# wheaton5/cellector

Measured on AMD Instinct MI355X. Metric: cell x locus log-likelihood evals/sec over full EM iterations (EM iters/sec in em_iters_per_s), higher is better.
Workload: dtype f64

## Files before the change

### cellector_amd/csrc/kernels_tiled.hip

```cpp
#include <hip/hip_ext.h>

#include "tiled.h"

__device__ __constant__ uint8_t T_A_OF[T_NCODE] = {1, 0, 2, 1, 0, 3, 2, 1, 0, 4, 3, 2, 1, 0};
__device__ __constant__ uint8_t T_R_OF[T_NCODE] = {0, 1, 0, 1, 2, 0, 1, 2, 3, 0, 1, 2, 3, 4};

struct ab_src_t {
    const double *s_alt, *s_ref, *alt_min, *ref_min;
    const uint8_t *mask;
    double2 *ab_out;
    double *xl_counters;
    uint32_t *d_counters, *tile_work;
    uint32_t n_work;
};
template <bool PAIRS>
__global__ __launch_bounds__(64 * TB_PARTS) void k_build_tables(uint64_t L, uint32_t nj, const double2 *__restrict__ ab,
                                                                const double *__restrict__ lf, double *__restrict__ tab,
                                                                ab_src_t src)
{
    if (src.s_alt && blockIdx.x == 0) {
        if (threadIdx.x < LC_COUNTERS) src.xl_counters[threadIdx.x] = 0.0;
        if (threadIdx.x < 8) src.d_counters[threadIdx.x] = 0u;
        for (uint32_t i = threadIdx.x; i < src.n_work; i += blockDim.x) src.tile_work[i] = 0u;
    }
    const int part = threadIdx.x >> 6;
    const uint64_t t = (uint64_t)blockIdx.x * 64 + (threadIdx.x & 63);
    if (t >= (uint64_t)nj * T_BL) return;
    const uint64_t chunk = t / T_BL, slot = t % T_BL;
    const uint64_t l = chunk * T_BLU + slot;
    double2 p = make_double2(-1.0, -1.0);
    if (slot < T_BLU && l < L) {
        if (src.s_alt) {
            p.x = (src.s_alt[l] + 1.0) - src.alt_min[l];
            p.y = (src.s_ref[l] + 1.0) - src.ref_min[l];
            if (!src.mask[l]) p.x = p.y = -1.0;
            if (part == 0) src.ab_out[l] = p;
        } else {
            p = ab[l];
        }
    }
    const bool live = p.x >= 0.0;
    double *row = tab + chunk * TAB_ELEMS + slot * T_LROW;
#define TB_PMF(W, A, R) row[W] = live ? dm_log_bb_pmf(lf, p.x, p.y, A, R) : 0.0
#define TB_EXP(N) row[T_NCODE + N - 1] = (PAIRS && live) ? dm_expected_log_pmf(lf, p.x, p.y, N) : 0.0
    switch (part) {
    case 0: TB_EXP(4u); TB_PMF(0, 1u, 0u); break;
    case 1: TB_EXP(3u); TB_PMF(1, 0u, 1u); break;
    case 2: TB_EXP(2u); TB_PMF(2, 2u, 0u); TB_PMF(3, 1u, 1u); break;
    case 3: TB_EXP(1u); TB_PMF(4, 0u, 2u); TB_PMF(5, 3u, 0u); break;
    case 4: TB_PMF(6, 2u, 1u); TB_PMF(7, 1u, 2u); TB_PMF(8, 0u, 3u); TB_PMF(9, 4u, 0u); break;
    default: TB_PMF(10, 3u, 1u); TB_PMF(11, 2u, 2u); TB_PMF(12, 1u, 3u); TB_PMF(13, 0u, 4u); break;
    }
#undef TB_PMF
#undef TB_EXP
}

#ifndef TILE_ABL
#define TILE_ABL 0
#endif
#ifndef TILE_PFD
#define TILE_PFD 2
#endif
#ifndef TILE_PFD_T2
#define TILE_PFD_T2 2
#endif
#ifndef TILE_PINNED
#define TILE_PINNED 1
#endif
#if TILE_ABL == 7
#define TILE_BARRIER() do { } while (0)
#else
#define TILE_BARRIER() asm volatile("s_waitcnt lgkmcnt(0)\n\ts_barrier" ::: "memory")
#endif

struct __attribute__((packed, aligned(4))) tile_u4 { uint32_t x, y, z, w; };

template <bool EXPECTED, int T_SB, class G = geo_reg>
__global__ __launch_bounds__(T_THREADS, 4) void k_tile_ll(uint32_t nb, uint32_t nj, uint32_t cpg, uint32_t groups,
                                                          uint32_t n_cols, uint32_t *__restrict__ work ,
                                                          const uint16_t *__restrict__ thdr,
                                                          const uint16_t *__restrict__ tiles,
                                                          const double *__restrict__ tab, uint64_t npad,
                                                          double *__restrict__ part_ll, double *__restrict__ part_ell)
{
    using tab_t = typename std::conditional<EXPECTED, double2, double>::type;
    constexpr uint32_t TAB_U = G::LROW * G::BL * sizeof(double) / 16;
    constexpr int NP = (TAB_U + T_THREADS - 1) / T_THREADS;
    static_assert(NP == 6, "table prefetch registers are written out by hand");
    __shared__ __attribute__((aligned(16))) double s_tab[G::LROW * G::BL];
    static_assert(G::LROW * G::BL % 2 == 0, "whole 16-byte units");
    __shared__ tab_t s_acc[T_SB * T_BC];
    __shared__ uint32_t s_col;
    const uint32_t tid = threadIdx.x, wv = tid >> 6, lane = tid & 63;
    const uint32_t g = blockIdx.x % groups;
    const uint32_t j0 = g * cpg, j1 = min(nj, j0 + cpg);
    if (j0 >= j1) return;
  for (;;) {
    if (tid == 0) s_col = atomicAdd(&work[g], 1u);
    __syncthreads();
    const uint32_t col = s_col;
    if (col >= n_cols) break;
    const uint32_t b0 = col * T_SB;
#pragma unroll
    for (int s = 0; s < T_SB; s++) {
        if constexpr (EXPECTED) s_acc[s * T_BC + tid] = make_double2(0.0, 0.0);
        else s_acc[s * T_BC + tid] = 0.0;
    }

    double2 p_t0, p_t1, p_t2, p_t3, p_t4, p_t5;
#define TABLE_PREFETCH(J)                                                                                        \
    do {                                                                                                         \
        const double2 *src__ = reinterpret_cast<const double2 *>(tab) + (uint64_t)(J) * TAB_U + tid;             \
        p_t0 = src__[0];                                                                                         \
        p_t1 = src__[T_THREADS];                                                                                 \
        p_t2 = src__[2 * T_THREADS];                                                                             \
        p_t3 = src__[3 * T_THREADS];                                                                             \
        p_t4 = src__[4 * T_THREADS];                                                                             \
        p_t5 = src__[5 * T_THREADS];                      \
    } while (0)

    struct row_t { tile_u4 lo, hi; uint32_t k; uint64_t base; };
    const uint32_t wv_s = (uint32_t)__builtin_amdgcn_readfirstlane((int)wv);
#define HDR_LOAD(H, J, S)            \
    do {                                                                                                         \
         \
         \
         \
        const uint32_t rot__ = (wv_s + 8u * ((uint32_t)(S) >> 1)) & 15u, sl__ = ((S) & 1u) ? 15u - rot__ : rot__; \
        if (TILE_ABL != 9 || first_rows)  \
        (H) = reinterpret_cast<const uint4 *>(thdr + ((uint64_t)min(b0 + (uint32_t)(S), nb - 1) * nj + (TILE_ABL == 10 ? j0 : (J))) * T_HDR)[sl__]; \
    } while (0)
#define ROW_LOAD(E, H)                                                                                           \
    do {                                                                                                         \
        (E).k = (SKIP_EMPTY && (H).w) ? 0u : (H).z;  \
        (E).base = ((uint64_t)(H).y << 32) | (H).x;                                                              \
         \
         \
        const char *sb__ = reinterpret_cast<const char *>(tiles + (E).base);                                     \
        const uint32_t off__ = __umul24(lane, ((H).z + 1u) * 2u);                      \
        if ((!(TILE_ABL == 2 || TILE_ABL == 9) || first_rows) && !(SKIP_EMPTY && (H).w)) {  \
            (E).lo = *reinterpret_cast<const tile_u4 *>(sb__ + off__);                                           \
            (E).hi = *reinterpret_cast<const tile_u4 *>(sb__ + ((H).z > 7u ? 16u : 0u) + off__);                 \
        }                                                                                                        \
    } while (0)

    constexpr bool SKIP_EMPTY = G::NLO != 1;
    constexpr uint32_t PFD = T_SB == 4 ? (uint32_t)(G::NLO == 1 ? TILE_PFD : TILE_PFD_T2) : 2u;
    static_assert(PFD >= 2 && PFD <= 4, "row buffers");
    uint4 h0, h1, h2, h3;
    row_t e0, e1, e2, e3;
    bool first_rows = true;
    TABLE_PREFETCH(j0);
    __builtin_amdgcn_sched_barrier(0);
#define HDR_STEP(H, T) HDR_LOAD(H, min(j0 + (uint32_t)(T) / T_SB, j1 - 1), (uint32_t)(T) % T_SB)
    HDR_STEP(h0, 0);
    HDR_STEP(h1, 1);
    if constexpr (PFD >= 3) HDR_STEP(h2, 2);
    if constexpr (PFD == 4) HDR_STEP(h3, 3);
    ROW_LOAD(e0, h0);
    ROW_LOAD(e1, h1);
    if constexpr (PFD >= 3) ROW_LOAD(e2, h2);
    if constexpr (PFD == 4) ROW_LOAD(e3, h3);
    HDR_STEP(h0, PFD);
    HDR_STEP(h1, PFD + 1);
    if constexpr (PFD >= 3) HDR_STEP(h2, PFD + 2);
    if constexpr (PFD == 4) HDR_STEP(h3, PFD + 3);
#undef HDR_STEP
    first_rows = false;

#if TILE_ABL == 1 || TILE_ABL == 5
#define TILE_LOOKUP(V, E16) do { if constexpr (EXPECTED) V = make_double2((double)(E16), 1.0); else V = (double)(E16); } while (0)
#elif TILE_ABL == 4
#define TILE_LOOKUP(V, E16)                                                                                      \
    do {                                                                                                         \
        const uint32_t b__ = (((E16) >> 4) & 127u) * 32u + (lane & 31u), c__ = (((E16) >> 5) & 127u) * 32u + (lane & 31u); \
        if constexpr (EXPECTED) V = make_double2(s_tab[b__], s_tab[c__ + 4096u]);                                \
        else V = s_tab[b__];                                                                                     \
    } while (0)
#else
#define TILE_LOOKUP(V, E16)                                                                                      \
    do {                                                                                                         \
        const uint32_t b__ = (((E16) >> G::SHIFT) & G::SMASK) * G::LROW;                                         \
        if constexpr (EXPECTED) V = make_double2(s_tab[b__ + ((E16) & G::CMASK)], s_tab[b__ + G::NCODE + ((E16) >> 14)]); \
        else V = s_tab[b__ + ((E16) & G::CMASK)];                                                                \
    } while (0)
#endif
#define TILE_RD(V, KK)                                                                                           \
    tab_t V;                                                                                                     \
    do {                                                                                                         \
        const uint32_t idx__ = (((KK) + 1) & 1) ? (w__[((KK) + 1) >> 1] >> 16) : (w__[((KK) + 1) >> 1] & 0xffffu); \
        TILE_LOOKUP(V, idx__);                                                                                   \
    } while (0)
#define TILE_ADD(V)                                                                                              \
    do {                                                                                                         \
        if constexpr (EXPECTED) { a_ll__ += (V).x; a_el__ += (V).y; }                                            \
        else a_ll__ += (V);                                                                                      \
    } while (0)
#if TILE_PINNED
#define TILE_PIN(V)                                                                                              \
    do {                                                                                                         \
        if constexpr (EXPECTED) asm volatile("" : "+v"((V).x), "+v"((V).y) : : "memory");                        \
        else asm volatile("" : "+v"(V) : : "memory");                                                            \
    } while (0)
#else
#define TILE_PIN(V) do { } while (0)
#endif
#define TILE_LEVEL(KA, KB, PA, PB, BODY)                                                                         \
    if (K__ > (KA)) {                                                                                            \
        TILE_RD(v##KA, KA); TILE_RD(v##KB, KB);                                                                  \
        TILE_PIN(PA); TILE_PIN(PB);                                                                              \
        TILE_ADD(PA); TILE_ADD(PB);                                                                              \
        BODY                                                                                                     \
    } else { TILE_ADD(PA); TILE_ADD(PB); }
#define TILE_STEP(S, E, H)                                                                                       \
    do {                                                                                                         \
         \
        const uint32_t w__[8] = {(E).lo.x, (E).lo.y, (E).lo.z, (E).lo.w, (E).hi.x, (E).hi.y, (E).hi.z, (E).hi.w}; \
        const uint32_t K__ = (uint32_t)__builtin_amdgcn_readfirstlane((int)(E).k);        \
        const uint64_t cur_base__ = (E).base;                                                                    \
        const uint32_t cell__ = w__[0] & 0xffffu;                                                                \
              \
        ROW_LOAD(E, H);                                                                                          \
        HDR_LOAD(H, min(j + ((S) + 2 * PFD) / T_SB, j1 - 1), ((S) + 2 * PFD) % T_SB);                            \
         \
          \
        if (!(SKIP_EMPTY && K__ == 0u)) {                                                                        \
        tab_t acc__;                                                                                             \
        if constexpr (TILE_ABL == 8) { if constexpr (EXPECTED) acc__ = make_double2(0.0, 0.0); else acc__ = 0.0; }        \
        else acc__ = s_acc[(S) * T_BC + (TILE_ABL == 6 ? tid : cell__)];                                         \
        double a_ll__ = 0.0, a_el__ = 0.0;                                                                       \
          \
        TILE_RD(v0, 0);                                                                                          \
        if (K__ > 1) {                                                                                           \
            TILE_RD(v1, 1); TILE_RD(v2, 2);                                                                      \
            TILE_PIN(v0);                                                                                        \
            TILE_ADD(v0);                                                                                        \
            TILE_LEVEL(3, 4, v1, v2,                                                                             \
            TILE_LEVEL(5, 6, v3, v4,                                                                             \
            TILE_LEVEL(7, 8, v5, v6,                                                                             \
            TILE_LEVEL(9, 10, v7, v8,                                                                            \
            TILE_LEVEL(11, 12, v9, v10,                                                                          \
            TILE_LEVEL(13, 14, v11, v12,                                                                         \
                TILE_ADD(v13); TILE_ADD(v14);                                                                    \
                for (uint32_t k = T_NE; k < K__; k++) {  \
                    tab_t v__;                                                                                   \
                    TILE_LOOKUP(v__, (uint32_t)(tiles + cur_base__ + lane * (K__ + 1u))[k + 1]);                 \
                    TILE_ADD(v__);                                                                               \
                } ))))))                                                                                         \
        } else TILE_ADD(v0);                                                                                     \
         \
         \
        if constexpr (EXPECTED) { acc__.x += a_ll__; acc__.y += a_el__; }                                        \
        else acc__ += a_ll__;                                                                                    \
        if (TILE_ABL != 8 || a_ll__ == 12345.678) s_acc[(S) * T_BC + (TILE_ABL == 6 ? tid : cell__)] = acc__;   \
        }                                                                                                        \
    } while (0)

    static_assert(T_SB == 2 || T_SB == 4, "even and odd steps use different pipeline buffers");
#if TILE_ABL == 3 || TILE_ABL == 5 || TILE_ABL == 7
#define TILE_STAGE_IF if (j == j0)
#define TILE_NEXT_TABLE() do { } while (0)
#else
#define TILE_STAGE_IF
#define TILE_NEXT_TABLE() TABLE_PREFETCH(min(j + 1, j1 - 1))
#endif
#define TILE_STAGE()                                                                                             \
    do {                                                                                                         \
// ... 236 lines not shown
                den *= fab;
                fa += isa ? 1.0 : 0.0;
                fb += isa ? 0.0 : 1.0;
                fab += 1.0;
            }
            lp = (lf[n] - lf[a] - lf[r]) + log(num * ov_rcp(den));
        } else {
            lp = ov_slow_log_pmf(lf, p.x, p.y, a, r);
        }
        s += lp;
        if (EXPECTED) e += ev;
    }
    s = group16_sum(s);
    if (EXPECTED) e = group16_sum(e);
    if (in && j == 0) {
        o_ll[row] = s;
        if (EXPECTED) o_ell[row] = e;
    }
}

template <bool EXPECTED>
__global__ __launch_bounds__(256) void k_t2_tables(uint32_t n_pairs, const uint32_t *__restrict__ plist ,
                                                   uint32_t n_sec, const uint32_t *__restrict__ slist ,
                                                   uint32_t gp, const double2 *__restrict__ ab, const double *__restrict__ lf,
                                                   double *__restrict__ tab2)
{
    if (blockIdx.x < gp) {
        const uint32_t i = blockIdx.x * 256 + threadIdx.x;
        if (i >= n_pairs) return;
        const uint32_t key = plist[i], l = key >> 5, c2 = key & 31u;
        const uint32_t n = 5u + (c2 >= 6u) + (c2 >= 13u) + (c2 >= 21u), r = c2 - t2_code(n, 0u), a = n - r;
        const double2 p = ab[l];
        double v = 0.0;
        if (p.x >= 0.0) {
            double num = 1.0, den = 1.0, fa = p.x, fb = p.y, fab = p.x + p.y;
#pragma unroll
            for (uint32_t k = 0; k < T2_NMAX; ++k) {
                const bool on = k < n, isa = k < a;
                num *= on ? (isa ? fa : fb) : 1.0;
                den *= on ? fab : 1.0;
                fa += isa ? 1.0 : 0.0;
                fb += (on && !isa) ? 1.0 : 0.0;
                fab += 1.0;
            }
            v = (lf[n] - lf[a] - lf[r]) + log(num / den);
        }
        tab2[(uint64_t)l * T2_ROW + t2_pos(n, r)] = v;
    } else if (EXPECTED) {
        const uint32_t i = (blockIdx.x - gp) * 256 + threadIdx.x;
        if (i >= n_sec) return;
        const uint32_t key = slist[i], l = key >> 3, sec = key & 7u;
        const uint32_t n = 5u + (sec >= 1u) + (sec >= 2u) + (sec >= 4u);
        const double2 p = ab[l];
        tab2[(uint64_t)l * T2_ROW + sec * 8u] = p.x >= 0.0 ? ov_expected_rec(p.x, p.y, n) : 0.0;
    }
}

template <bool EXPECTED, class G>
__global__ __launch_bounds__(256) void k_t2c_tables(uint64_t L, uint32_t gp, const double2 *__restrict__ ab, const double *__restrict__ lf,
                                                    double *__restrict__ tabc)
{
    constexpr uint64_t ELEMS = (uint64_t)G::LROW * G::BL;
    if (blockIdx.x < gp) {
        const uint64_t i = (uint64_t)blockIdx.x * 256 + threadIdx.x;
        const uint64_t l = i / G::NCODE;
        if (l >= L) return;
        const uint32_t c2 = (uint32_t)(i % G::NCODE);
        const uint32_t n = 5u + (c2 >= 6u) + (c2 >= 13u) + (c2 >= 21u), r = c2 - t2_code(n, 0u), a = n - r;
        const double2 p = ab[l];
        double v = 0.0;
        if (p.x >= 0.0) {
            double num = 1.0, den = 1.0, fa = p.x, fb = p.y, fab = p.x + p.y;
#pragma unroll
            for (uint32_t k = 0; k < T2_NMAX; ++k) {
                const bool on = k < n, isa = k < a;
                num *= on ? (isa ? fa : fb) : 1.0;
                den *= on ? fab : 1.0;
                fa += isa ? 1.0 : 0.0;
                fb += (on && !isa) ? 1.0 : 0.0;
                fab += 1.0;
            }
            v = (lf[n] - lf[a] - lf[r]) + log(num / den);
        }
        tabc[(l / G::BLU) * ELEMS + (l % G::BLU) * G::LROW + c2] = v;
    } else if (EXPECTED) {
        constexpr uint32_t NE = G::NHI - G::NLO + 1;
        const uint64_t i = (uint64_t)(blockIdx.x - gp) * 256 + threadIdx.x;
        const uint64_t l = i / NE;
        if (l >= L) return;
        const uint32_t n = G::NLO + (uint32_t)(i % NE);
        const double2 p = ab[l];
        tabc[(l / G::BLU) * ELEMS + (l % G::BLU) * G::LROW + G::NCODE + (n - G::NLO)] = p.x >= 0.0 ? ov_expected_rec(p.x, p.y, n) : 0.0;
    }
}

template <bool EXPECTED>
__global__ __launch_bounds__(256) void k_t2_tile_add(uint64_t n_rows, uint32_t groups, uint64_t npad, const double *__restrict__ part_ll,
                                                     const double *__restrict__ part_ell, double *__restrict__ o_ll,
                                                     double *__restrict__ o_ell)
{
    const uint64_t row = (uint64_t)blockIdx.x * 256 + threadIdx.x;
    if (row >= n_rows) return;
    double s = 0.0, e = 0.0;
    for (uint32_t g = 0; g < groups; g++) {
        s += part_ll[(uint64_t)g * npad + row];
        if (EXPECTED) e += part_ell[(uint64_t)g * npad + row];
    }
    o_ll[row] += s;
    if (EXPECTED) o_ell[row] += e;
}

template <bool EXPECTED>
__global__ __launch_bounds__(64) void k_t2_cell(uint64_t n_rows, const uint64_t *__restrict__ ell_ptr, const uint64_t *__restrict__ ell,
                                                const double *__restrict__ tab2, double *__restrict__ o_ll, double *__restrict__ o_ell)
{
  const uint64_t n_grp = (n_rows + 63) >> 6;
  for (uint64_t grp = blockIdx.x; grp < n_grp; grp += gridDim.x) {
    const uint64_t row = grp * 64 + threadIdx.x;
    if (row >= n_rows) continue;
    double s = 0.0, e = 0.0;
    const uint64_t base = ell_ptr[grp] + (row & 63), end = ell_ptr[grp + 1];
    constexpr int U = 4;
    for (uint64_t i = base; i < end; i += (uint64_t)U * 64) {
        uint64_t en[U];
        double lp[U], ev[U];
#pragma unroll
        for (int u = 0; u < U; u++) en[u] = i + (uint64_t)u * 64 < end ? ell[i + (uint64_t)u * 64] : OVF_PAD;
#pragma unroll
        for (int u = 0; u < U; u++) {
            const uint32_t r = ENT_REF(en[u]), n = ENT_ALT(en[u]) + r;
            const bool ok = en[u] != OVF_PAD && t2_total(n);
#ifdef T2_ABL
            const uint64_t at = (uint64_t)(ENT_IDX(en[u]) & 1023u) * T2_ROW + t2_pos(ok ? n : T2_NMIN, ok ? r : 0u);
#else
            const uint64_t at = (uint64_t)ENT_IDX(en[u]) * T2_ROW + t2_pos(ok ? n : T2_NMIN, ok ? r : 0u);
#endif
            lp[u] = ok ? tab2[at] : 0.0;
            if (EXPECTED) ev[u] = ok ? tab2[at & ~7ull] : 0.0;
        }
#pragma unroll
        for (int u = 0; u < U; u++) {
            s += lp[u];
            if (EXPECTED) e += ev[u];
        }
    }
    o_ll[row] = s;
    if (EXPECTED) o_ell[row] = e;
  }
}

__global__ __launch_bounds__(256) void k_t2_minority(const uint32_t *__restrict__ tc, int valid, uint64_t nloc,
                                                     const uint32_t *__restrict__ minlist, const uint32_t *__restrict__ chg,
                                                     const uint64_t *__restrict__ ovf_ptr, const uint64_t *__restrict__ ovf_ent,
                                                     uint32_t *__restrict__ cnt2)
{
    const uint32_t n_a = valid ? tc[1] : tc[0], n = valid ? n_a + tc[2] : n_a;
    const uint32_t j = threadIdx.x % LF_LANES;
    const uint32_t ng = gridDim.x * (256 / LF_LANES);
    for (uint32_t k = (blockIdx.x * 256 + threadIdx.x) / LF_LANES; k < n; k += ng) {
        const uint32_t cell = !valid ? minlist[k] : k < n_a ? chg[k] : chg[nloc - 1 - (k - n_a)];
        const uint32_t inc = k < n_a ? 1u : ~0u;
        for (uint64_t i = ovf_ptr[cell] + j, end = ovf_ptr[cell + 1]; i < end; i += LF_LANES) {
            const uint64_t en = ovf_ent[i];
            const uint32_t r = ENT_REF(en), t = ENT_ALT(en) + r;
            if (t2_total(t)) atomicAdd(&cnt2[(uint64_t)ENT_IDX(en) * T2_CSTRIDE + t2_code(t, r)], inc);
        }
    }
}

__global__ __launch_bounds__(256) void k_ovx_values(uint64_t n_ovx, const uint32_t *__restrict__ ovx_locus, const uint64_t *__restrict__ ovx_ent,
                                                    const double2 *__restrict__ ab, const double *__restrict__ lf, double *__restrict__ lp_out)
{
    const uint64_t i = (uint64_t)blockIdx.x * 256 + threadIdx.x;
    if (i >= n_ovx) return;
    const uint64_t en = ovx_ent[i];
// ... 366 lines not shown
        s_len[tid] = p_n;
        __syncthreads();
        LR_PREFETCH(kb + LR_THREADS);
        constexpr int SPW = 64 / LR_GROUP;
        constexpr int NQ = 16;
        for (uint32_t q0 = 0; q0 < 64 / SPW; q0 += NQ) {
            uint32_t e[NQ];
#pragma unroll
            for (int u = 0; u < NQ; u++) {
                const uint32_t seg = wv * 64 + (q0 + u) * SPW + grp;
                e[u] = gl < s_len[seg] ? (uint32_t)c4r[s_beg[seg] + gl] : 0xffffu;
            }
#pragma unroll
            for (int u = 0; u < NQ; u++) LR_COUNT(e[u]);
            for (int u = 0; u < NQ; u++) {
                const uint32_t seg = wv * 64 + (q0 + u) * SPW + grp;
                const uint32_t sn = s_len[seg];
                const uint64_t sb = s_beg[seg];
                for (uint32_t j = gl + LR_GROUP; j < sn; j += LR_GROUP) {
                    const uint32_t x = (uint32_t)c4r[sb + j];
                    LR_COUNT(x);
                }
            }
        }
        __syncthreads();
    }
#undef LR_PREFETCH
#undef LR_COUNT
    __syncthreads();
    const uint64_t nl = min((uint64_t)LR_LOCI, L - l0);
    uint32_t *dst = reinterpret_cast<uint32_t *>(reinterpret_cast<uint16_t *>(hist_min) + ((uint64_t)sub * L + l0) * 16);
    for (uint32_t i = tid; i < nl * 8; i += LR_THREADS) {
        const uint32_t lo = i >> 3, c0 = (i & 7u) * 2u;
        uint32_t v = 0;
#pragma unroll
        for (uint32_t h = 0; h < 2; h++) {
            const uint32_t code = c0 + h, idx = code * LR_ROW + lo;
            if (code < (uint32_t)T_NCODE) v |= ((s_hist[idx >> 1] >> ((idx & 1u) * 16u)) & 0xffffu) << (16u * h);
        }
        dst[i] = v;
    }
}

template <bool INLINE_OVF>
__global__ __launch_bounds__(256) void k_locus_finalize(uint64_t L, int locus_mode, int valid, uint64_t nloc, uint32_t n_sub, uint32_t sub_cap,
                                                        const uint32_t *__restrict__ tc,
                                                        const uint32_t *__restrict__ hist_min, uint32_t *__restrict__ tally,
                                                        const uint32_t *__restrict__ flag_bits,
                                                        const uint32_t *__restrict__ hist_all,
                                                        const double *__restrict__ tab, uint32_t tab_stride,
                                                        const uint8_t *__restrict__ mask,
                                                        const uint64_t *__restrict__ ovc_ptr ,
                                                        const uint64_t *__restrict__ ovc_ent,
                                                        const double *__restrict__ ovf_lp ,
                                                        const double *__restrict__ otab, const double *__restrict__ lf,
                                                        const double2 *__restrict__ ab, double *__restrict__ out,
                                                        const uint32_t *__restrict__ cnt2 ,
                                                        const uint32_t *__restrict__ hist_all2, const uint32_t *__restrict__ pmask2,
                                                        const double *__restrict__ tab2,
                                                        uint8_t *__restrict__ mask_next ,
                                                        uint32_t *__restrict__ n_filtered)
{
    const TallyPlan tp = tally_plan(locus_mode, valid, tc, nloc, n_sub, sub_cap);
    const uint32_t n_planes = tp.s_a + tp.s_r;
    const uint32_t j = threadIdx.x % LF_LANES;
    const uint64_t l_raw = ((uint64_t)blockIdx.x * 256 + threadIdx.x) / LF_LANES;
    const bool in = l_raw < L;
    const uint64_t l = in ? l_raw : L - 1;
    const bool live = mask[l] != 0;
    uint64_t obeg = 0, oend = 0;
    if (ovc_ptr) { obeg = ovc_ptr[l]; oend = ovc_ptr[l + 1]; }
    double cmin = 0.0, cmaj = 0.0;
    uint32_t nmin = 0;
    uint64_t amin = 0, rmin = 0;
    if (j < T_NCODE) {
        uint32_t cnt = tp.fresh ? 0u : tally[l * 16 + j];
        if (n_planes) {
            const uint16_t *h16 = reinterpret_cast<const uint16_t *>(hist_min);
            for (uint32_t p = 0; p < tp.s_a; p++) cnt += h16[((uint64_t)p * L + l) * 16 + j];
            for (uint32_t p = tp.s_a; p < n_planes; p++) cnt -= h16[((uint64_t)p * L + l) * 16 + j];
        }
        if (in && (n_planes || tp.fresh)) tally[l * 16 + j] = cnt;
        const uint32_t h_all = hist_all[l * T_NCODE + j];
        const double t_code = tab[(l / T_BLU) * TAB_ELEMS + (l % T_BLU) * T_LROW + j];
        amin = (uint64_t)cnt * T_A_OF[j];
        rmin = (uint64_t)cnt * T_R_OF[j];
        if (live) {
            nmin = cnt;
            cmin = (double)cnt * t_code;
            cmaj = (double)(h_all - cnt) * t_code;
        }
    }
    if (cnt2) {
        const uint32_t pm = pmask2[l];
#pragma unroll
        for (uint32_t h = 0; h < 2; h++) {
            const uint32_t c2 = j + h * LF_LANES;
            if (!((pm >> c2) & 1u)) continue;
            const uint32_t h_all = hist_all2[l * T2_CSTRIDE + c2];
            const uint32_t cnt = cnt2[l * T2_CSTRIDE + c2];
            const uint32_t n2 = 5u + (c2 >= 6u) + (c2 >= 13u) + (c2 >= 21u), r2 = c2 - t2_code(n2, 0u);
            const double t_code = tab2[l * T2_ROW + t2_pos(n2, r2)];
            amin += (uint64_t)cnt * (n2 - r2);
            rmin += (uint64_t)cnt * r2;
            if (live) {
                nmin += cnt;
                cmin += (double)cnt * t_code;
                cmaj += (double)(h_all - cnt) * t_code;
            }
        }
    }
    const double *orow = otab + l * OV_ROW;
    for (uint64_t i0 = obeg + j; i0 < oend; i0 += 4 * LF_LANES) {
        uint64_t en[4];
        double lp[4];
        uint32_t w[4];
#pragma unroll
        for (int u = 0; u < 4; u++) {
            const uint64_t i = i0 + (uint64_t)u * LF_LANES;
            en[u] = i < oend ? ovc_ent[i] : ~0ull;
            lp[u] = (!INLINE_OVF && i < oend) ? ovf_lp[i] : 0.0;
        }
#pragma unroll
        for (int u = 0; u < 4; u++) w[u] = en[u] != ~0ull ? flag_bits[ENT_IDX(en[u]) >> 5] : 0u;
#pragma unroll
        for (int u = 0; u < 4; u++) {
            if (!INLINE_OVF) break;
            lp[u] = 0.0;
            if (en[u] == ~0ull || !live) continue;
            const uint32_t a = ENT_ALT(en[u]), r = ENT_REF(en[u]), n = a + r;
            if (n == 0) lp[u] = 0.0;
            else if (n < (uint32_t)OV_NT)
                lp[u] = (lf[n] - lf[a] - lf[r]) + (orow[a] + orow[OV_NT + r] - orow[2 * OV_NT + n]);
            else {
                const double2 p = ab[l];
                lp[u] = ov_slow_log_pmf(lf, p.x, p.y, a, r);
            }
        }
#pragma unroll
        for (int u = 0; u < 4; u++) {
            if (en[u] == ~0ull) continue;
            const bool minority = ((w[u] >> (ENT_IDX(en[u]) & 31)) & 1u) != 0;
            if (minority) { amin += ENT_ALT(en[u]); rmin += ENT_REF(en[u]); }
            if (live) {
                if (minority) { cmin += lp[u]; nmin++; } else cmaj += lp[u];
            }
        }
    }
    cmin = group16_sum(cmin);
    cmaj = group16_sum(cmaj);
    nmin = group16_sum(nmin);
    amin = group16_sum(amin);
    rmin = group16_sum(rmin);
    if (in && j == 0) {
        out[LB_CONTRIB_MIN * L + l] = cmin;
        out[LB_CONTRIB_MAJ * L + l] = cmaj;
        out[LB_CELLS_MIN * L + l] = (double)nmin;
        out[LB_ALT_MIN * L + l] = (double)amin;
        out[LB_REF_MIN * L + l] = (double)rmin;
        if (mask_next) {
            const double fn = (double)nmin;
            const double per_cell = fn != 0.0 ? cmin / fn : 0.0;
            uint8_t m = mask[l];
            if (per_cell < -80.0) {
                m = 0;
                atomicAdd(n_filtered, 1u);
            }
// ... 493 lines not shown
```

### cellector_amd/csrc/kernels_tiled_build.hip

```cpp
#include "tiled.h"

__device__ __forceinline__ uint64_t row_lower_bound(const uint64_t *__restrict__ ent, uint64_t lo, uint64_t hi, uint32_t locus)
{
    while (lo < hi) {
        const uint64_t mid = (lo + hi) >> 1;
        if (ENT_IDX(ent[mid]) < locus) lo = mid + 1; else hi = mid;
    }
    return lo;
}

template <class G>
__device__ __forceinline__ bool geo_take(uint64_t e)
{
    const uint32_t n = ENT_ALT(e) + ENT_REF(e);
    return n - G::NLO <= G::NHI - G::NLO;
}
template <class G>
__device__ __forceinline__ uint16_t geo_encode(uint64_t e, uint32_t j)
{
    const uint32_t r = ENT_REF(e), n = ENT_ALT(e) + r;
    const uint32_t code = G::NLO == 1 ? ent_code(e) : t2_code(n, r);
    return (uint16_t)(((n - G::NLO) << 14) | ((ENT_IDX(e) - j * G::BLU) << G::SHIFT) | code);
}
template <bool FILL, class G = geo_reg>
// ... 16 lines not shown
    if (cl < T_BC / 64) s_kmax[cl] = 0;
    uint64_t lo = 0, hi = 0;
    uint32_t len = 0;
    if (row < nloc) {
        const uint64_t beg = csr_ptr[row], end = csr_ptr[row + 1];
        if (toff) {
            lo = beg + toff[row * (nj + 1) + j];
            hi = beg + toff[row * (nj + 1) + j + 1];
        } else {
            lo = row_lower_bound(csr_ent, beg, end, j * G::BLU);
            hi = row_lower_bound(csr_ent, lo, end, (j + 1u) * G::BLU);
        }
        for (uint64_t i = lo; i < hi; i++) len += geo_take<G>(csr_ent[i]) ? 1u : 0u;
    }
    __syncthreads();
    const uint32_t bin = min(len, (uint32_t)TB_BINS - 1u);
    uint32_t within = 0;
    {
        unsigned long long todo = ~0ull;
        while (todo) {
            const int src = __ffsll((long long)todo) - 1;
            const uint32_t v = (uint32_t)__shfl((int)bin, src, 64);
            const unsigned long long m = __ballot(bin == v);
            if (bin == v) within = (uint32_t)__popcll(m & ((1ull << lane) - 1ull));
            if ((int)lane == src) s_cnt[wv][v] = (uint32_t)__popcll(m);
            todo &= ~m;
        }
    }
    __syncthreads();
    if (cl < TB_BINS) {
        uint32_t tot = 0;
        for (int w = 0; w < T_BC / 64; w++) tot += s_cnt[w][cl];
        uint32_t inc = tot;
#pragma unroll
        for (int off = 1; off < 64; off <<= 1) {
            const uint32_t o = __shfl_up(inc, off, 64);
            if ((int)cl >= off) inc += o;
        }
        s_base[cl] = inc - tot;
    }
    __syncthreads();
    uint32_t rank = s_base[bin] + within;
    for (uint32_t w = 0; w < wv; w++) rank += s_cnt[w][bin];
    const uint32_t dw = rank >> 6, dl = rank & 63;
    atomicMax(&s_kmax[dw], len);
    __syncthreads();
    if (cl == 0) {
        uint32_t acc = 0;
        for (int w = 0; w < T_BC / 64; w++) {
            s_sbase[w] = acc;
            acc += 64u * ((s_kmax[w] | 1u) + 1u);
        }
        s_sbase[T_BC / 64] = acc;
    }
    __syncthreads();
    if (!FILL) {
        if (cl == 0) tile_elems[t] = (uint64_t)s_sbase[T_BC / 64];
        return;
    }
    const uint64_t tbase = tile_elems[t];
    uint16_t *hp = thdr + t * T_HDR;
    if (cl < T_BC / 64) {
        uint32_t *hd = reinterpret_cast<uint32_t *>(hp) + 4 * cl;
        const uint64_t first = tbase + s_sbase[cl];
        hd[0] = (uint32_t)first;
        hd[1] = (uint32_t)(first >> 32);
        hd[2] = s_kmax[cl] | 1u;
        hd[3] = s_kmax[cl] == 0u;
    }
    const uint32_t K = s_kmax[dw] | 1u;
    uint16_t *dst = tiles + tbase + s_sbase[dw] + dl * (K + 1u);
    dst[0] = (uint16_t)cl;
    uint32_t k = 0;
    for (uint64_t i = lo; i < hi; i++) {
        const uint64_t e = csr_ent[i];
        if (geo_take<G>(e)) dst[1 + k++] = geo_encode<G>(e, j);
    }
    for (; k < K; k++) dst[1 + k] = (uint16_t)(G::BLU << G::SHIFT);
}

#define TBO_ROUNDS 4
__device__ __forceinline__ void tbo_banks(uint32_t e, uint32_t *a, uint32_t *b)
{
    const uint32_t base = ((e >> 4) & 1023u) * (uint32_t)T_LROW;
    *a = (base + (e & 15u)) & 31u;
    *b = (base + (uint32_t)T_NCODE + (e >> 14)) & 31u;
}
__device__ uint32_t tile_lane_assign(uint16_t *slice , uint32_t Kw, uint32_t lane, uint32_t cnt, uint32_t *scr)
{
#define TLA_SYNC() asm volatile("s_waitcnt lgkmcnt(0)" ::: "memory")
    const uint32_t cls = (uint32_t)slice[lane * (Kw + 1u)] & 15u;
    const unsigned long long lt = (1ull << lane) - 1ull;
    uint32_t t = 0;
#pragma unroll
    for (uint32_t c = 0; c < 16u; c++) {
        const unsigned long long m = __ballot(cls == c);
        if (c < cls) t += (uint32_t)__popcll(m);
        else if (c == cls) t += (uint32_t)__popcll(m & lt);
    }
    const uint32_t g = t & 3u, pp = ((t >> 2) + ((g & 1u) ? 8u : 0u)) & 15u;
    const uint32_t l0 = pp < 4u ? pp : (pp < 8u ? pp + 8u : pp + 12u);
    const uint32_t l1 = pp < 8u ? pp + 4u : (pp < 12u ? pp + 8u : pp + 16u);
    const uint32_t dst = ((g & 1u) ? l1 : l0) + ((g & 2u) ? 32u : 0u);
    scr[dst] = lane;
    scr[64 + dst] = cnt;
    TLA_SYNC();
    const uint32_t src = scr[lane], cnt_new = scr[64 + lane];
    for (uint32_t k = 0; k <= Kw; k++) {
        const uint16_t v = slice[src * (Kw + 1u) + k];
        TLA_SYNC();
        slice[lane * (Kw + 1u) + k] = v;
        TLA_SYNC();
    }
    return cnt_new;
#undef TLA_SYNC
}

#define TBO_WIN 4
__device__ void tile_bank_order(uint16_t *row , uint32_t K, uint32_t cnt ,
                                uint32_t lane, uint32_t *scr )
{
    const uint32_t h = lane >> 5;
    uint32_t *ld_a = scr + h * 64, *ld_b = ld_a + 32, *win_a = scr + 128 + h * 64, *win_b = win_a + 32;
#define TBO_SYNC() asm volatile("s_waitcnt lgkmcnt(0)" ::: "memory")
    if (K <= 1u) return;
    for (uint32_t k = 0; k + 1u < K; k++) {
        if (__ballot(k + 1u < cnt) == 0ull) break;
        scr[lane] = 0u; scr[64 + lane] = 0u;
        uint32_t e[TBO_WIN], ca[TBO_WIN], cb[TBO_WIN];
#pragma unroll
        for (uint32_t u = 0; u < (uint32_t)TBO_WIN; u++) {
            e[u] = k + u < cnt ? (uint32_t)row[k + u] : 0xffffffffu;
            tbo_banks(e[u], &ca[u], &cb[u]);
        }
        bool open = k < cnt;
        TBO_SYNC();
        for (uint32_t rd = 0; rd < (uint32_t)TBO_ROUNDS; rd++) {
            if (__ballot(open) == 0ull) break;
            scr[128 + lane] = ~0u; scr[192 + lane] = ~0u;
            uint32_t cost[TBO_WIN];
#pragma unroll
            for (uint32_t u = 0; u < (uint32_t)TBO_WIN; u++) cost[u] = ld_a[ca[u]] + ld_b[cb[u]];
            uint32_t best = 0, bc = cost[0];
#pragma unroll
            for (uint32_t u = 1; u < (uint32_t)TBO_WIN; u++)
                if (e[u] != 0xffffffffu && cost[u] < bc) { bc = cost[u]; best = u; }
            uint32_t ba = ca[0], bb = cb[0];
#pragma unroll
            for (uint32_t u = 1; u < (uint32_t)TBO_WIN; u++)
                if (best == u) { ba = ca[u]; bb = cb[u]; }
            TBO_SYNC();
            if (open) {
                atomicMin(&win_a[ba], lane);
                atomicMin(&win_b[bb], lane);
            }
            TBO_SYNC();
            if (open && (rd == (uint32_t)TBO_ROUNDS - 1u || (win_a[ba] == lane && win_b[bb] == lane))) {
                if (best) {
                    uint32_t eb = e[0];
#pragma unroll
                    for (uint32_t u = 1; u < (uint32_t)TBO_WIN; u++)
                        if (best == u) eb = e[u];
                    row[k] = (uint16_t)eb;
                    row[k + best] = (uint16_t)e[0];
                }
                atomicAdd(&ld_a[ba], 1u);
                atomicAdd(&ld_b[bb], 1u);
                open = false;
            }
// ... 633 lines not shown
```

### cellector_amd/csrc/tiled.h

```cpp
#pragma once
#include <algorithm>
#include <initializer_list>
#include <type_traits>

#include "ctx.h"
#include "device_math.h"

#define T_K 4
#define T_NCODE 14
#ifndef T_LROW
#define T_LROW 18
#endif
#ifndef T_BL
#define T_BL 640
#endif
#define T_BLU (T_BL - 1)
#define T_BC 1024
#define T_THREADS 1024
static_assert(T_BC == T_ROWS_PER_TILE, "cellector_engine_info derives the lookup count from this");
#define T_SB_MAX 4
#define T_GROUPS_MAX 64
static_assert(T_GROUPS_MAX == CELLECTOR_TILE_WORK_STRIDE, "k_alpha_beta resets the counters with this stride");
#define T_GROUPS 8
#define T_NE 15
#define T_NULL ((uint16_t)(T_BLU << 4))
#define T_HDR 128
#define TAB_ELEMS ((uint64_t)T_LROW * T_BL)

__device__ __forceinline__ bool ent_regular(uint64_t e)
{
    const uint32_t n = ENT_ALT(e) + ENT_REF(e);
    return n >= 1u && n <= (uint32_t)T_K;
}
__device__ __forceinline__ uint32_t ent_code(uint64_t e)
{
    const uint32_t r = ENT_REF(e), n = ENT_ALT(e) + r;
    return n * (n + 1u) / 2u - 1u + r;
}

#define TB_PARTS 6

struct geo_reg {
    static constexpr uint32_t LROW = T_LROW, BL = T_BL, NCODE = T_NCODE, SHIFT = 4, SMASK = 1023u, CMASK = 15u;
    static constexpr uint32_t BLU = BL - 1, NLO = 1, NHI = T_K;
};
template <int NMAX>
struct geo_t2 {
    static_assert(NMAX == 6 || NMAX == 8, "tier-2 tile geometries");
    static constexpr uint32_t NCODE = NMAX == 8 ? 30 : 13, NE = NMAX - 4, LROW = NCODE + NE;
    static constexpr uint32_t BL = NMAX == 8 ? 339 : 768, SHIFT = NMAX == 8 ? 5 : 4, SMASK = NMAX == 8 ? 511u : 1023u,
                              CMASK = NMAX == 8 ? 31u : 15u;
    static constexpr uint32_t BLU = BL - 1, NLO = 5, NHI = NMAX;
};

#define LF_LANES 16
#define OV_NT 18
#define OV_NE 17
#define OV_FAST_N DM_CHUNK
#define OV_ROW 128
#define OV_EOFF 64
#define OV_REC 8
#define OVF_PAD (~0ull)

#define T2_NMIN 5u
#define T2_NMAX 8u
#define T2_NCODE 30
#define T2_CSTRIDE 32
#define T2_ROW 48
static_assert(T2_NMAX == (unsigned)OV_FAST_N, "the tier lists take the totals above tier 2");
__device__ __forceinline__ bool t2_total(uint32_t n) { return n - T2_NMIN <= T2_NMAX - T2_NMIN; }
__device__ __forceinline__ uint32_t t2_code(uint32_t n, uint32_t r) { return n * (n + 1u) / 2u - 15u + r; }
__device__ __forceinline__ uint32_t t2_pos(uint32_t n, uint32_t r)
{
    const uint32_t hi = r >= 7u ? 1u : 0u;
    return ((n - T2_NMIN) + (n == 8u ? 1u : 0u) + hi) * 8u + 1u + (hi ? r - 7u : r);
}
__device__ __forceinline__ int ovf_tier(uint64_t en)
{
    const uint32_t n = ENT_ALT(en) + ENT_REF(en);
    return n <= (uint32_t)OV_FAST_N ? -1 : (n <= (uint32_t)OV_NE ? 0 : 1);
}

template <int EB>
__device__ __forceinline__ void c4_read1(const uint32_t *__restrict__ base, uint64_t i, uint32_t *cell, uint32_t *code)
{
    if (EB == 32) {
        const uint32_t x = base[i];
        *cell = x & 0x0fffffffu;
        *code = x >> 28;
    } else {
        const uint8_t *b = reinterpret_cast<const uint8_t *>(base) + 3 * i;
        const uint32_t v = (uint32_t)b[0] | ((uint32_t)b[1] << 8) | ((uint32_t)b[2] << 16);
        *cell = v & 0xfffffu;
        *code = v >> 20;
    }
}
template <int EB>
__device__ __forceinline__ void c4_write1(uint32_t *__restrict__ base, uint64_t i, uint32_t cell, uint32_t code)
{
    if (EB == 32) {
        base[i] = cell | (code << 28);
    } else {
        uint8_t *b = reinterpret_cast<uint8_t *>(base) + 3 * i;
        const uint32_t v = cell | (code << 20);
        b[0] = (uint8_t)v; b[1] = (uint8_t)(v >> 8); b[2] = (uint8_t)(v >> 16);
    }
}
#define LM_NUM 1
#define LM_DEN 8

#define LR_LOCI 4096
#define LR_SUB_MAX 16
#define LR_THREADS 1024
#define LR_GROUP 64
#define LR_ROW (LR_LOCI + 2)
#define LT_CELLS 64
#define TB_BINS 64
#define TB_STAGE (24 * 1024)

static inline unsigned gcap(uint64_t n, unsigned per_block, unsigned cap = 1u << 20)
{
    uint64_t g = (n + per_block - 1) / per_block;
    if (g < 1) g = 1;
    if (g > cap) g = cap;
    return (unsigned)g;
}

template <class F>
static inline void with_bool(bool b, F &&f)
{
    if (b) f(std::true_type());
    else f(std::false_type());
}

struct CountedPtr { uint64_t *ptr, *total; };
template <class Pass, class Payload>
// ... 12 lines not shown
```

Baseline: 1060 billion.

## Store regular-tier lookup tables in code-major layout instead of slot-major

Adds tab_pmf/tab_exp index helpers and switches the regular-tier per-chunk log-pmf table to a code-major (structure-of-arrays) layout by default, with the expected-log terms placed first and each code's values contiguous across slots. The builder, the tile lookup macro, the tally read and the LDS bank-assignment helper all use the new indexing. The aim is to change LDS bank mapping and write coalescing for the gathered table lookups in the tiled likelihood kernel. Bank-conflict behaviour of the lane-assignment heuristic shifts with it, and the tier-2 geometries stay slot-major.

```diff
diff --git a/cellector_amd/csrc/kernels_tiled.hip b/cellector_amd/csrc/kernels_tiled.hip
--- a/cellector_amd/csrc/kernels_tiled.hip
+++ b/cellector_amd/csrc/kernels_tiled.hip
@@ -40,9 +40,9 @@
         }
     }
     const bool live = p.x >= 0.0;
-    double *row = tab + chunk * TAB_ELEMS + slot * T_LROW;
-#define TB_PMF(W, A, R) row[W] = live ? dm_log_bb_pmf(lf, p.x, p.y, A, R) : 0.0
-#define TB_EXP(N) row[T_NCODE + N - 1] = (PAIRS && live) ? dm_expected_log_pmf(lf, p.x, p.y, N) : 0.0
+    double *img = tab + chunk * TAB_ELEMS;
+#define TB_PMF(W, A, R) img[tab_pmf<geo_reg>((uint32_t)slot, W)] = live ? dm_log_bb_pmf(lf, p.x, p.y, A, R) : 0.0
+#define TB_EXP(N) img[tab_exp<geo_reg>((uint32_t)slot, N - 1)] = (PAIRS && live) ? dm_expected_log_pmf(lf, p.x, p.y, N) : 0.0
     switch (part) {
     case 0: TB_EXP(4u); TB_PMF(0, 1u, 0u); break;
     case 1: TB_EXP(3u); TB_PMF(1, 0u, 1u); break;
@@ -180,9 +180,9 @@
 #else
 #define TILE_LOOKUP(V, E16)                                                                                      \
     do {                                                                                                         \
-        const uint32_t b__ = (((E16) >> G::SHIFT) & G::SMASK) * G::LROW;                                         \
-        if constexpr (EXPECTED) V = make_double2(s_tab[b__ + ((E16) & G::CMASK)], s_tab[b__ + G::NCODE + ((E16) >> 14)]); \
-        else V = s_tab[b__ + ((E16) & G::CMASK)];                                                                \
+        const uint32_t s__ = ((E16) >> G::SHIFT) & G::SMASK;                                                     \
+        if constexpr (EXPECTED) V = make_double2(s_tab[tab_pmf<G>(s__, (E16) & G::CMASK)], s_tab[tab_exp<G>(s__, (E16) >> 14)]); \
+        else V = s_tab[tab_pmf<G>(s__, (E16) & G::CMASK)];                                                       \
     } while (0)
 #endif
 #define TILE_RD(V, KK)                                                                                           \
@@ -585,7 +585,7 @@
             }
             v = (lf[n] - lf[a] - lf[r]) + log(num / den);
         }
-        tabc[(l / G::BLU) * ELEMS + (l % G::BLU) * G::LROW + c2] = v;
+        tabc[(l / G::BLU) * ELEMS + tab_pmf<G>((uint32_t)(l % G::BLU), c2)] = v;
     } else if (EXPECTED) {
         constexpr uint32_t NE = G::NHI - G::NLO + 1;
         const uint64_t i = (uint64_t)(blockIdx.x - gp) * 256 + threadIdx.x;
@@ -593,7 +593,7 @@
         if (l >= L) return;
         const uint32_t n = G::NLO + (uint32_t)(i % NE);
         const double2 p = ab[l];
-        tabc[(l / G::BLU) * ELEMS + (l % G::BLU) * G::LROW + G::NCODE + (n - G::NLO)] = p.x >= 0.0 ? ov_expected_rec(p.x, p.y, n) : 0.0;
+        tabc[(l / G::BLU) * ELEMS + tab_exp<G>((uint32_t)(l % G::BLU), n - G::NLO)] = p.x >= 0.0 ? ov_expected_rec(p.x, p.y, n) : 0.0;
     }
 }
 
@@ -1126,7 +1126,7 @@
         }
         if (in && (n_planes || tp.fresh)) tally[l * 16 + j] = cnt;
         const uint32_t h_all = hist_all[l * T_NCODE + j];
-        const double t_code = tab[(l / T_BLU) * TAB_ELEMS + (l % T_BLU) * T_LROW + j];
+        const double t_code = tab[(l / T_BLU) * TAB_ELEMS + tab_pmf<geo_reg>((uint32_t)(l % T_BLU), j)];
         amin = (uint64_t)cnt * T_A_OF[j];
         rmin = (uint64_t)cnt * T_R_OF[j];
         if (live) {
diff --git a/cellector_amd/csrc/kernels_tiled_build.hip b/cellector_amd/csrc/kernels_tiled_build.hip
--- a/cellector_amd/csrc/kernels_tiled_build.hip
+++ b/cellector_amd/csrc/kernels_tiled_build.hip
@@ -122,9 +122,9 @@
 #define TBO_ROUNDS 4
 __device__ __forceinline__ void tbo_banks(uint32_t e, uint32_t *a, uint32_t *b)
 {
-    const uint32_t base = ((e >> 4) & 1023u) * (uint32_t)T_LROW;
-    *a = (base + (e & 15u)) & 31u;
-    *b = (base + (uint32_t)T_NCODE + (e >> 14)) & 31u;
+    const uint32_t slot = (e >> geo_reg::SHIFT) & geo_reg::SMASK;
+    *a = tab_pmf<geo_reg>(slot, e & geo_reg::CMASK) & 31u;
+    *b = tab_exp<geo_reg>(slot, e >> 14) & 31u;
 }
 __device__ uint32_t tile_lane_assign(uint16_t *slice , uint32_t Kw, uint32_t lane, uint32_t cnt, uint32_t *scr)
 {
diff --git a/cellector_amd/csrc/tiled.h b/cellector_amd/csrc/tiled.h
--- a/cellector_amd/csrc/tiled.h
+++ b/cellector_amd/csrc/tiled.h
@@ -40,9 +40,13 @@
 
 #define TB_PARTS 6
 
+#ifndef TILE_CM
+#define TILE_CM 1
+#endif
 struct geo_reg {
     static constexpr uint32_t LROW = T_LROW, BL = T_BL, NCODE = T_NCODE, SHIFT = 4, SMASK = 1023u, CMASK = 15u;
     static constexpr uint32_t BLU = BL - 1, NLO = 1, NHI = T_K;
+    static constexpr bool CODE_MAJOR = TILE_CM != 0;
 };
 template <int NMAX>
 struct geo_t2 {
@@ -51,7 +55,18 @@
     static constexpr uint32_t BL = NMAX == 8 ? 339 : 768, SHIFT = NMAX == 8 ? 5 : 4, SMASK = NMAX == 8 ? 511u : 1023u,
                               CMASK = NMAX == 8 ? 31u : 15u;
     static constexpr uint32_t BLU = BL - 1, NLO = 5, NHI = NMAX;
+    static constexpr bool CODE_MAJOR = false;
 };
+template <class G>
+__host__ __device__ __forceinline__ constexpr uint32_t tab_pmf(uint32_t slot, uint32_t code)
+{
+    return G::CODE_MAJOR ? (G::LROW - G::NCODE + code) * G::BL + slot : slot * G::LROW + code;
+}
+template <class G>
+__host__ __device__ __forceinline__ constexpr uint32_t tab_exp(uint32_t slot, uint32_t ne)
+{
+    return G::CODE_MAJOR ? ne * G::BL + slot : slot * G::LROW + G::NCODE + ne;
+}
 
 #define LF_LANES 16
 #define OV_NT 18
```

New measurement: 1085 billion (median of 6 runs). +2.4%, better.
